# Jeffrey-Ede/AI-CV-Automation-Elect-Micr

Measured on AMD Instinct MI355X. Metric: megapixels/sec restored (512x512x1 bs=32), higher is better.
Workload: dtype bf16x3 (split-bf16 MFMA inputs, fp32 accumulate and activations)

## Files before the change

ai-cv-automation-elect-micr_amd/_lib.py:

```python
from __future__ import annotations

import ctypes as C
import os

PKG_DIR = os.path.dirname(os.path.abspath(__file__))
LIB_PATH = os.environ.get("EMD_LIB_PATH") or os.path.join(PKG_DIR, "libemdenoise.so")

EMD_OK = 0
EMD_K_SYMMETRIC = 1

_c_float_p = C.c_void_p

class PackJob(C.Structure):
    _fields_ = [("w", C.c_void_p), ("hi", C.c_void_p), ("lo", C.c_void_p), ("tap_sel", C.c_ulonglong), ("total", C.c_long),
                ("first_block", C.c_long), ("n_blocks", C.c_long), ("ntaps", C.c_int), ("cin", C.c_int), ("cout", C.c_int),
                ("cout_major", C.c_int), ("cpad", C.c_int), ("pad_", C.c_int)]


class KFusedJob(C.Structure):
    _fields_ = [("theta", C.c_void_p), ("adam_m", C.c_void_p), ("adam_v", C.c_void_p), ("step", C.c_void_p),
                ("params_out", C.c_void_p), ("losses", C.c_void_p), ("width", C.c_int), ("depth", C.c_int)]


SIGNATURES = {
# ... 336 lines not shown
    "emd_propagate_f64": (C.c_int, [C.c_void_p, C.c_int, C.c_int, C.c_int, C.c_int, C.c_void_p, C.c_double, C.c_double, C.c_double,
                                    C.c_void_p, C.c_void_p, C.c_size_t, C.c_void_p]),
    "emd_exitwave_workspace_bytes": (C.c_size_t, [C.c_int] * 3),
    "emd_exitwave_reconstruct_f64": (C.c_int, [C.c_void_p, C.c_int, C.c_int, C.c_int, C.c_void_p, C.c_double, C.c_double, C.c_double,
                                               C.c_int, C.c_int, C.c_void_p, C.c_void_p, C.c_void_p, C.c_void_p, C.c_size_t, C.c_void_p]),
    "emd_hanning_window_f64": (C.c_int, [C.c_int, C.c_void_p, C.c_void_p, C.c_void_p]),
    "emd_phase_correlate_workspace_bytes": (C.c_size_t, [C.c_int] * 3),
    "emd_phase_correlate_f64": (C.c_int, [C.c_void_p, C.c_void_p, C.c_int, C.c_int, C.c_int, C.c_void_p, C.c_void_p, C.c_void_p, C.c_size_t,
                                          C.c_void_p]),
    "emd_stack_centres_f64": (C.c_int, [C.c_void_p, C.c_int, C.c_int, C.c_void_p, C.c_void_p]),
    "emd_crop_stack_f32": (C.c_int, [C.c_void_p, C.c_int, C.c_int, C.c_void_p, C.c_int, C.c_float, C.c_void_p, C.c_void_p]),
    "emd_warp_affine_f32": (C.c_int, [C.c_void_p, C.c_int, C.c_int, C.c_int, C.c_void_p, C.c_int, C.c_float, C.c_void_p, C.c_void_p]),
    "emd_mi_samples_u32": (C.c_int, [C.c_int, C.c_int, C.c_int, C.c_uint64, C.c_void_p, C.c_void_p]),
    "emd_mattes_mi_workspace_bytes": (C.c_size_t, [C.c_int] * 5),
    "emd_mattes_mi_f64": (C.c_int, [C.c_void_p, C.c_void_p, C.c_int, C.c_int, C.c_int, C.c_void_p, C.c_void_p, C.c_int, C.c_int, C.c_void_p,
                                    C.c_void_p, C.c_void_p, C.c_void_p, C.c_size_t, C.c_void_p]),
    "emd_affine_normals_f64": (C.c_int, [C.c_int, C.c_int, C.c_int, C.c_uint64, C.c_void_p, C.c_void_p]),
    "emd_affine_register_f64": (C.c_int, [C.c_void_p, C.c_void_p, C.c_int, C.c_int, C.c_int, C.c_void_p, C.c_int, C.c_int, C.c_double,
                                          C.c_double, C.c_double, C.c_uint64, C.c_void_p, C.c_int, C.c_int, C.c_void_p, C.c_int, C.c_int,
                                          C.c_void_p, C.c_void_p, C.c_size_t, C.c_void_p]),
    "emd_affine_chain_f64": (C.c_int, [C.c_void_p, C.c_int, C.c_int, C.c_void_p, C.c_void_p]),
    "emd_affine_limits_i32": (C.c_int, [C.c_void_p, C.c_int, C.c_int, C.c_int, C.c_void_p, C.c_void_p]),
    "emd_psiart_ctf_f64": (C.c_int, [C.c_int, C.c_int, C.c_void_p, C.c_void_p, C.c_double, C.c_double, C.c_double, C.c_void_p, C.c_void_p]),
    "emd_psiart_workspace_bytes": (C.c_size_t, [C.c_int] * 2),
    "emd_psiart_loss_grad_f64": (C.c_int, [C.c_void_p, C.c_int, C.c_int] + [C.c_void_p] * 5 + [C.c_double] * 3 + [C.c_int] +
                                 [C.c_void_p] * 5 + [C.c_void_p, C.c_size_t, C.c_void_p]),
    "emd_psiart_step_f64": (C.c_int, [C.c_void_p, C.c_int, C.c_int] + [C.c_void_p] * 5 + [C.c_double] * 3 + [C.c_int] +
                            [C.c_void_p] * 8 + [C.c_double] * 3 + [C.c_void_p] * 5 + [C.c_void_p, C.c_size_t, C.c_void_p]),
}

DEV_SIGNATURES = {
    "emd_debug_knob": (C.c_int, [C.c_char_p, C.c_long]),
    "emd_debug_reduce_final_cl": (C.c_int, [C.c_int]),
    "emd_debug_split_variant": (None, [C.c_int]),
    "emd_debug_split_stamps": (None, [C.c_void_p]),
    "emd_debug_sep_stamps": (None, [C.c_void_p]),
    "emd_debug_sepgemm_stamps": (None, [C.c_void_p]),
    "emd_debug_stream_copy_f32": (C.c_int, [C.c_void_p, C.c_void_p, C.c_long, C.c_void_p]),
    "emd_debug_mfma_peak_bf16": (C.c_int, [C.c_void_p, C.c_void_p, C.c_int, C.c_int, C.c_void_p]),
}

_lib = None


class EmdError(RuntimeError):
    pass


def load():
    global _lib
    if _lib is not None:
        return _lib
    if not os.path.exists(LIB_PATH):
        raise EmdError(
            f"{LIB_PATH} not found: build the HIP extension first "
            "(python ai-cv-automation-elect-micr_amd/build.py, or __graft_entry__.build()). "
            "There is no CPU fallback for this path.")
    import torch

    lib = C.CDLL(LIB_PATH)
    for name, (res, args) in list(SIGNATURES.items()) + list(DEV_SIGNATURES.items()):
        fn = getattr(lib, name)
        fn.restype = res
        fn.argtypes = args
    _lib = lib
    for kv in filter(None, os.environ.get("EMD_KNOBS", "").split(",")):
# ... 37 lines not shown
```

ai-cv-automation-elect-micr_amd/csrc/emd_common.hip:

```cpp
#include <cstring>

#include "emd_common.hpp"

namespace emd {

static thread_local char g_err[512] = "";

void set_error(const char* fmt, ...) {
    va_list ap;
    va_start(ap, fmt);
    vsnprintf(g_err, sizeof(g_err), fmt, ap);
    va_end(ap);
}

Knobs g_knobs;

}

extern "C" int emd_version(void) { return EMD_VERSION; }

extern "C" const char* emd_last_error(void) { return emd::g_err; }

extern "C" int emd_debug_reduce_final_cl(int nslab) { return emd::reduce_final_cl(nslab); }

extern "C" int emd_debug_knob(const char* name, long value) {
    using emd::g_knobs;
    struct { const char* n; int* v; } tab[] = {
        {"sep_pipe", &g_knobs.sep_pipe}, {"sep_pipe2", &g_knobs.sep_pipe2}, {"sep_stamp_wave", &g_knobs.sep_stamp_wave}, {"sep_mode", &g_knobs.sep_mode}, {"sep_tpw", &g_knobs.sep_tpw}, {"sep_ablate", &g_knobs.sep_ablate}, {"sep_nw", &g_knobs.sep_nw}, {"sep_xcd", &g_knobs.sep_xcd},
        {"sep_wide", &g_knobs.sep_wide}, {"sep_wres", &g_knobs.sep_wres}, {"nt_mask", &g_knobs.nt_mask}, {"deconv_direct", &g_knobs.deconv_direct}, {"epi_width", &g_knobs.epi_width}, {"split_lead", &g_knobs.split_lead}, {"dw_xcd", &g_knobs.dw_xcd},
        {"dw_th", &g_knobs.dw_th},       {"split_variant", &g_knobs.split_variant}, {"split_narrow", &g_knobs.split_narrow}, {"split_wide", &g_knobs.split_wide}, {"conv3_pipe", &g_knobs.conv3_pipe}, {"wgrad_msplit", &g_knobs.wgrad_msplit}, {"wgrad_tile", &g_knobs.wgrad_tile}, {"sep_gen_pipe", &g_knobs.sep_gen_pipe}, {"fold_final", &g_knobs.fold_final}, {"up_fused", &g_knobs.up_fused}, {"exitwave_composed", &g_knobs.exitwave_composed}, {"resize_generic", &g_knobs.resize_generic},
    };
    if (!name) return -1;
    for (auto& e : tab)
        if (!strcmp(name, e.n)) { *e.v = (int)value; return 0; }
    return -1;
}
```

ai-cv-automation-elect-micr_amd/csrc/emd_common.hpp:

```cpp
#pragma once

#include <hip/hip_runtime.h>

#include <cstdarg>
#include <cstdint>
#include <cstdio>

#include "../../include/emdenoise.h"

namespace emd {

void set_error(const char* fmt, ...) __attribute__((format(printf, 1, 2)));

inline int fail(int code, const char* what) {
    set_error("%s", what);
    return code;
}

inline int check_launch(const char* kernel) {
    hipError_t e = hipGetLastError();
    if (e != hipSuccess) {
        set_error("%s: %s", kernel, hipGetErrorString(e));
        return EMD_E_LAUNCH;
    }
// ... 31 lines not shown
    bool optional;
    bool input;
};

inline int check_ranges(const char* who, const Range* r, int n, const char* aligned, const size_t* workspace_bytes = nullptr) {
    for (int i = 0; i < n; ++i)
        if (!r[i].p && !r[i].optional) {
            set_error("%s: null pointer", who);
            return EMD_E_INVALID;
        }
    if (workspace_bytes && *workspace_bytes < r[0].n) {
        set_error("%s: workspace too small (%zu bytes, needs %zu)", who, *workspace_bytes, r[0].n);
        return EMD_E_INVALID;
    }
    for (int i = 0; i < n; ++i)
        if (r[i].p && (reinterpret_cast<uintptr_t>(r[i].p) & (r[i].align - 1))) {
            set_error("%s: %s", who, aligned);
            return EMD_E_ALIGN;
        }
    for (int i = 0; i < n; ++i)
        for (int j = i + 1; j < n; ++j)
            if (r[i].p && r[j].p && !(r[i].input && r[j].input) && overlap(r[i].p, r[i].n, r[j].p, r[j].n)) {
                set_error("%s: the outputs and the workspace may overlap neither one another nor the inputs", who);
                return EMD_E_INVALID;
            }
    return EMD_OK;
}

constexpr int kWave = 64;

struct Knobs {
    int sep_pipe = 1;
    int sep_pipe2 = 0;
    int sep_gen_pipe = 0;
    int sep_mode = -1;
    int sep_nw = 0;
    int sep_ablate = 0;
    int sep_tpw = 0;
    int sep_xcd = 1;
    int sep_wide = 1;
    int sep_wres = 1;
    int fold_final = 1;
    int up_fused = 1;
    int epi_width = 0;
    int deconv_direct = 3;
    int nt_mask = 7;
    int dw_xcd = 1;
    int dw_th = 0;
    int split_narrow = 1;
    int split_lead = 2;
    int split_wide = 0;
    int conv3_pipe = 1;
    int split_variant = -1;
    int exitwave_composed = 0;
    int resize_generic = 0;
    int sep_stamp_wave = 0;
    int wgrad_msplit = 0;
    int wgrad_tile = 0;
    long long* sep_stamps = nullptr;
};
extern Knobs g_knobs;

inline long reduce_rows_per_slab(long npix) {
    long r = (npix + 511) / 512;
    return r < 64 ? 64 : r;
}
// ... 13 lines not shown
```

ai-cv-automation-elect-micr_amd/csrc/sep_fused.hip:

```cpp
#include <cstdlib>
#include <type_traits>

#include "sep_params.hpp"

using namespace emd;

namespace {

__device__ __attribute__((aligned(16))) float g_zero_px[4096];

inline int sep_nt() { return (g_knobs.nt_mask >> 1) & 1; }
inline int sep_xcd() { return g_knobs.sep_xcd; }

template <int BN, int PASSES, bool GEN, int TH = 8, bool DUAL = false, bool WRES = false>
__global__ __launch_bounds__(256, 2) void sep_fused_kernel(const SepParams p) {
    constexpr int TW = 16, BM = TH * TW, BK = 32;
    constexpr int PH = TH + 2, PW = TW + 2, NPX = PH * PW;
    constexpr int PLD = 40;
    constexpr int LDK = BK + 8;
    constexpr int WN = BN / 64, WM = 4 / WN;
    constexpr int TM = BM / WM / 32, TN = BN / WN / 32;
    constexpr int NPL = PASSES == 3 ? 2 : 1;
    constexpr int P_PASSES = (NPX * 8 + 255) / 256;
    constexpr int W_PASSES = BN / 64;
// ... 904 lines not shown

extern "C" int emd_sep3x3_fused_gen9_f32(const float* img, const float* w9, const float* gen_a, const float* gen_t, int gen_act,
                                         const float* dw, const uint16_t* whi, const uint16_t* wlo, const float* scale1,
                                         const float* shift1, const float* scale2, const float* shift2, const float* res,
                                         int ldres, float* y, int ldy, int B, int H, int W, int Cin, int Cout, int act,
                                         int precision, int reflect, emd_stream_t stream) {
    EMD_REQUIRE(img && w9 && gen_a && gen_t && dw && whi && wlo && scale1 && shift1 && y, EMD_E_INVALID,
                "emd_sep3x3_fused_gen9_f32: null pointer");
    EMD_REQUIRE((scale2 == nullptr) == (shift2 == nullptr), EMD_E_INVALID, "emd_sep3x3_fused_gen9_f32: scale2/shift2 pair");
    EMD_REQUIRE(B >= 0 && H >= 1 && W >= 1, EMD_E_INVALID, "emd_sep3x3_fused_gen9_f32: bad shape");
    EMD_REQUIRE(gen_act == EMD_ACT_RELU6 && !reflect && precision == 3 && emd_sep3x3_fused_gen9_supported(H, W, Cin, Cout),
                EMD_E_UNSUPPORTED,
                "emd_sep3x3_fused_gen9_f32: needs relu6 generation, zero padding, split-bf16, H%8==0, W%16==0, Cin 32 or 64, Cout%4==0, "
                "Cout<=64 (use emd_cin1_f32 + emd_sep3x3_fused_gen_f32)");
    EMD_REQUIRE(B <= 65535, EMD_E_UNSUPPORTED, "emd_sep3x3_fused_gen9_f32: B > 65535");
    EMD_REQUIRE(9L * W * (ldy > ldres ? ldy : ldres) < (1L << 31), EMD_E_UNSUPPORTED,
                "emd_sep3x3_fused_gen9_f32: 9 image rows of the output must span fewer than 2^31 floats");
    EMD_REQUIRE(ldy % 4 == 0 && ldy >= Cout && (!res || (ldres % 4 == 0 && ldres >= Cout)), EMD_E_ALIGN,
                "emd_sep3x3_fused_gen9_f32: pixel strides must be multiples of 4 and >= the channel count");
    EMD_REQUIRE(emd::aligned16(gen_a) && emd::aligned16(gen_t) && emd::aligned16(dw) && emd::aligned16(whi) && emd::aligned16(wlo) &&
                    emd::aligned16(y) && (!res || emd::aligned16(res)) && emd::aligned16(scale1) && emd::aligned16(shift1) &&
                    (!scale2 || (emd::aligned16(scale2) && emd::aligned16(shift2))),
                EMD_E_ALIGN, "emd_sep3x3_fused_gen9_f32: pointers (but img, w9) must be 16-byte aligned");
    if (B == 0) return EMD_OK;
    SepParams p{};
    p.x = img; p.dw = dw; p.Whi = whi; p.Wlo = wlo; p.y = y; p.res = res;
    p.scale1 = scale1; p.shift1 = shift1; p.scale2 = scale2; p.shift2 = shift2;
    p.H = H; p.W = W; p.Cin = Cin; p.Cpad = (Cin + kBK - 1) / kBK * kBK; p.N = Cout;
    p.ldx = 1; p.ldy = ldy; p.ldres = ldres; p.act = act; p.stride = 1;
    p.gen_a = gen_a; p.gen_t = gen_t; p.gen_act = gen_act; p.gen_w9 = w9;
    return launch_gen9(p, B, static_cast<hipStream_t>(stream));
}

extern "C" void emd_debug_sep_stamps(void* buf) { g_knobs.sep_stamps = static_cast<long long*>(buf); }

extern "C" int emd_sep3x3_dual_supported(int H, int W, int Cin, int Cout, int Cout2) {
    const bool wide = Cout > 64 || Cout2 > 64;
    return H % (wide ? 4 : 8) == 0 && W % 16 == 0 && Cin % 32 == 0 && Cin >= 32 && Cin <= 4096 && Cout % 4 == 0 && Cout2 % 4 == 0 &&
           Cout >= 4 && Cout2 >= 4 && Cout <= 128 && Cout2 <= 128;
}

extern "C" int emd_sep3x3_dual_preferred(int H, int W, int Cin, int Cout, int Cout2) {
    if (!emd_sep3x3_dual_supported(H, W, Cin, Cout, Cout2)) return 0;
    if (Cout <= 64 && Cout2 <= 64) return 1;
    return H % 8 == 0 && W % 32 == 0;
}

extern "C" int emd_sep3x3_dual_f32(const float* x, int ldx, const float* dw, const uint16_t* whi, const uint16_t* wlo,
                                   const float* scale1, const float* shift1, float* y, int ldy, const uint16_t* w2hi,
                                   const uint16_t* w2lo, const float* scale_b, const float* shift_b, float* y2, int ldy2, int B, int H,
                                   int W, int Cin, int Cout, int Cout2, int act, emd_stream_t stream) {
    EMD_REQUIRE(x && dw && whi && wlo && scale1 && shift1 && y && w2hi && w2lo && scale_b && shift_b && y2, EMD_E_INVALID,
                "emd_sep3x3_dual_f32: null pointer");
    EMD_REQUIRE(B >= 0 && H >= 1 && W >= 1, EMD_E_INVALID, "emd_sep3x3_dual_f32: bad shape");
    EMD_REQUIRE(emd_sep3x3_dual_supported(H, W, Cin, Cout, Cout2), EMD_E_UNSUPPORTED,
                "emd_sep3x3_dual_f32: needs H%8==0 (H%4==0 above 64 output channels), W%16==0, Cin%32==0, Cout%4==0, Cout<=128 (both outputs)");
    EMD_REQUIRE(B <= 65535, EMD_E_UNSUPPORTED, "emd_sep3x3_dual_f32: B > 65535");
    EMD_REQUIRE(9L * W * (ldy > ldy2 ? ldy : ldy2) < (1L << 31), EMD_E_UNSUPPORTED,
                "emd_sep3x3_dual_f32: 9 image rows of an output must span fewer than 2^31 floats");
    EMD_REQUIRE(ldx % 4 == 0 && ldx >= Cin && ldy % 4 == 0 && ldy >= Cout && ldy2 % 4 == 0 && ldy2 >= Cout2, EMD_E_ALIGN,
                "emd_sep3x3_dual_f32: pixel strides must be multiples of 4 and >= the channel count");
    EMD_REQUIRE(emd::aligned16(x) && emd::aligned16(dw) && emd::aligned16(whi) && emd::aligned16(wlo) && emd::aligned16(w2hi) &&
                    emd::aligned16(w2lo) && emd::aligned16(y) && emd::aligned16(y2) && emd::aligned16(scale1) && emd::aligned16(shift1) &&
                    emd::aligned16(scale_b) && emd::aligned16(shift_b),
                EMD_E_ALIGN, "emd_sep3x3_dual_f32: pointers must be 16-byte aligned");
    EMD_REQUIRE(y != y2, EMD_E_INVALID, "emd_sep3x3_dual_f32: the two outputs alias");
// ... 11 lines not shown
```

ai-cv-automation-elect-micr_amd/csrc/sep_params.hpp:

```cpp
#pragma once

#include "mfma_common.hpp"

namespace emd {

struct SepParams {
    const float* x;
    const float* dw;
    const uint16_t* Whi;
    const uint16_t* Wlo;
    float* y;
    const float* res;
    const float* scale1;
    const float* shift1;
    const float* scale2;
    const float* shift2;
    int H, W, Cin, Cpad, N;
    int ldx, ldy, ldres, act;
    int stride;
    int reflect;
    int tpw;
    const float* gen_a;
    const float* gen_t;
    int gen_act;
    int rg_stride;
    union { const uint16_t* W2hi; const float* rg_x; const float* gen_w9; };
    union { const uint16_t* W2lo; const float* fold_w; };
    union { float* y2; float* fold_z; };
    union { const float* scale_b; const float* rg_a; };
    union { const float* shift_b; const float* rg_t; };
    int N2;
    union { int ldy2; int fold; };
    int out_split;
    int rg_ld;
    long long* stamps;
    int nt;
    int ablate;
    int xcd;
    int rg_act;
};
inline bool folded(const SepParams& p) { return p.N2 == 0 && p.fold != 0; }
static_assert(sizeof(SepParams) == 232, "SepParams: the rg_* fields fill padding and share storage; see above before adding a field");

bool sep_pipe_covers(const SepParams& p, int precision);
int sep_pipe_launch(const SepParams& p, int B, hipStream_t st);
bool sep_pipe2_covers(const SepParams& p);
int sep_pipe2_launch(const SepParams& p, int B, hipStream_t st);

}
```

ai-cv-automation-elect-micr_amd/csrc/sep_pipe.hip:

```cpp
#include <type_traits>

#include "sep_params.hpp"

namespace {

using namespace emd;

__device__ __attribute__((aligned(16))) float g_zero_pipe[4096];

template <int BN, bool DUAL, int MODE, bool OSPLIT, int NW = 8, int STRIDE = 1, int EPI = 1, bool GEN = false, bool RGEN = false, bool FOLD = false>
__global__ __launch_bounds__(NW * 64, 2) void sep_pipe_kernel(const SepParams p) {
    constexpr int TW = STRIDE == 2 ? 16 : 4 * NW, TH = STRIDE == 2 ? 4 : 8, BM = TH * TW;
    constexpr int PW = STRIDE * TW + 3 - STRIDE, PH = STRIDE * TH + 3 - STRIDE, PWS = PW | 1;
    constexpr bool WPAD = PWS > PW && PH >= 9;
    constexpr int NPATCH = PH * PWS, NSLOT = WPAD ? NPATCH : NPATCH + 9;
    constexpr int WK0 = WPAD ? PW : NPATCH, WKS = WPAD ? PWS : 1;
    constexpr int NPIECE = (NSLOT + 7) / 8;
    constexpr int PP = (NPIECE + NW - 1) / NW;
    constexpr int STAGE = NPIECE * 1024;
    constexpr int A_BYTES = BM * 128, B_ONE = BN * 128;
    constexpr bool BDBL = BN <= 128 && NW == 8;
    constexpr int PB = BN / 8 / NW;
    constexpr bool LEAD2 = MODE == 0;
    constexpr int WN = STRIDE == 2 ? 4 : BN / 64, WM = NW / WN, TM = BM / WM / 32, TN = BN / WN / 32;
// ... 799 lines not shown
}

namespace emd {

static bool use_nw4(const SepParams& p) {
    if (g_knobs.sep_nw == 8 || p.stride == 2) return false;
    return p.N2 > 0 ? (p.N <= 64 && p.N2 <= 64) : (p.N <= 128 && !(p.out_split && p.N <= 64));
}

bool sep_pipe_covers(const SepParams& p, int precision) {
    if (!g_knobs.sep_pipe || precision != 3) return false;
    if (folded(p))
        return p.stride == 1 && p.H % 8 == 0 && p.W % 16 == 0 && p.Cin % 32 == 0 && p.Cin >= 32 && p.Cin <= 4064 && p.N == 64 && p.N2 == 0 &&
               !p.out_split && !p.gen_a && !p.rg_stride && !p.reflect && g_knobs.sep_nw != 8;
    if (p.gen_a)
        return g_knobs.sep_gen_pipe && p.stride == 1 && p.H % 8 == 0 && p.W % 16 == 0 && (p.Cin == 32 || p.Cin == 64) && p.N <= 64 && p.N2 == 0 &&
               !p.out_split && !p.res && g_knobs.sep_nw != 8;
    if (p.rg_stride && (p.stride != 2 || p.N2 > 0 || p.N > 128 || p.res || p.reflect)) return false;
    if (p.stride == 2)
        return p.H % 8 == 0 && p.W % 32 == 0 && p.Cin % 32 == 0 && p.Cin >= 32 && p.Cin <= 4064 && p.N2 == 0 && !p.out_split && p.N <= 256;
    if (p.H % 8 != 0 || p.W % (use_nw4(p) ? 16 : 32) != 0 || p.Cin % 32 != 0 || p.Cin < 32 || p.Cin > 4064) return false;
    if (p.N2 > 0) return p.N <= 128 && p.N2 <= 128 && !p.out_split && !p.res && !p.scale2;
    if (p.out_split && p.N <= 64) return false;
    return p.N <= 256;
}

static bool use_pipe2(const SepParams& p) {
    if (p.gen_a || p.rg_stride || folded(p)) return false;
    if (!g_knobs.sep_pipe2 || g_knobs.sep_ablate || g_knobs.sep_nw == 4 || !sep_pipe2_covers(p)) return false;
    if (g_knobs.sep_pipe2 == 2) return true;
    return p.N2 > 0 && (p.N > 64 || p.N2 > 64);
}

int sep_pipe_launch(const SepParams& p, int B, hipStream_t st) {
    if (use_pipe2(p)) return sep_pipe2_launch(p, B, st);
    SepParams q = p;
    const bool s2 = p.stride == 2;
    const int nw = (p.gen_a || folded(p) || (!s2 && use_nw4(p))) ? 4 : 8, tw = s2 ? 16 : 4 * nw, th = s2 ? 4 : 8;
    const int Ho = p.H / (s2 ? 2 : 1), Wo = p.W / (s2 ? 2 : 1);
    const int tiles_w = Wo / tw;
    const long wgs1 = (long)tiles_w * (Ho / th) * B;
    int tpw = 1;
    for (int t = 8; t >= 2; t >>= 1)
        if (tiles_w % t == 0 && wgs1 / t >= 1024 * (8 / nw)) { tpw = t; break; }
    if (g_knobs.sep_tpw > 0 && tiles_w % g_knobs.sep_tpw == 0) tpw = g_knobs.sep_tpw;
    q.tpw = tpw;
    q.stamps = g_knobs.sep_stamps;
    q.ablate = g_knobs.sep_ablate;
    const dim3 grid(tiles_w / tpw, Ho / th, B);
    q.xcd = g_knobs.sep_xcd && ((long)grid.x * grid.y * grid.z) % 8 == 0;
    const int mode = g_knobs.sep_mode >= 0 ? g_knobs.sep_mode : ((nw == 4 || p.res) ? 1 : 0);
    if (folded(p)) {
        if (mode == 1) hipLaunchKernelGGL((sep_pipe_kernel<64, false, 1, false, 4, 1, 1, false, false, true>), grid, dim3(256), 0, st, q);
        else hipLaunchKernelGGL((sep_pipe_kernel<64, false, 0, false, 4, 1, 1, false, false, true>), grid, dim3(256), 0, st, q);
        return emd::check_launch("sep_pipe_kernel<folded final conv>");
    }
    if (p.gen_a) {
        if (g_knobs.epi_width == 4) hipLaunchKernelGGL((sep_pipe_kernel<64, false, 1, false, 4, 1, 4, true>), grid, dim3(256), 0, st, q);
        else hipLaunchKernelGGL((sep_pipe_kernel<64, false, 1, false, 4, 1, 1, true>), grid, dim3(256), 0, st, q);
        return emd::check_launch("sep_pipe_kernel<generated input>");
    }
    if (p.rg_stride) {
        hipLaunchKernelGGL((sep_pipe_kernel<128, false, 1, false, 8, 2, 1, false, true>), grid, dim3(512), 0, st, q);
        return emd::check_launch("sep_pipe_kernel<stride 2, generated residual>");
    }
    const int epi = g_knobs.epi_width ? g_knobs.epi_width : ((p.res && p.N > 128) ? 4 : 1);
    return epi == 4 ? launch_epi<4>(p, q, grid, mode, nw, st) : launch_epi<1>(p, q, grid, mode, nw, st);
}
// ... 3 lines not shown
```

ai-cv-automation-elect-micr_amd/csrc/sep_pipe2.hip:

```cpp
#include "sep_params.hpp"

namespace {

using namespace emd;

__device__ __attribute__((aligned(16))) float g_zero_pipe2[4096];

typedef __attribute__((ext_vector_type(2))) float f32x2v;

template <int BN, bool DUAL, bool OSPLIT, int EPI>
__global__ __launch_bounds__(512, 2) void sep_pipe2_kernel(const SepParams p) {
    constexpr int NW = 8, TW = 32, TH = 8, BM = TH * TW;
    constexpr int PW = TW + 2, PH = TH + 2, PWS = PW | 1;
    constexpr int NPATCH = PH * PWS, NSLOT = NPATCH;
    constexpr int WK0 = PW, WKS = PWS;
    constexpr int NPIECE = (NSLOT + 7) / 8, PP = (NPIECE + NW - 1) / NW, STAGE = NPIECE * 1024;
    constexpr int A_HALF = BM * 64, B_HALF = BN * 64;
    constexpr int A_OFF = 2 * STAGE, B_OFF = A_OFF + 2 * A_HALF, C_OFF = B_OFF + 2 * B_HALF, SMEM = C_OFF + 16 * BN;
    constexpr int NBP = BN / 16;
    constexpr int PB = NBP >= NW ? NBP / NW : 1;
    constexpr int WN = BN / 64, WM = NW / WN, TM = BM / WM / 32, TN = 2;
    constexpr int E = 16 / EPI * TM * TN;
    constexpr bool RPRE = TM == 1 && !DUAL;
    constexpr int R = RPRE ? 16 / EPI * TM * TN : 0;
    static_assert(SMEM <= 160 * 1024 && PP >= 2, "shape");
    static_assert(!(DUAL && OSPLIT), "split32 output: one-output instances only");
    __shared__ __attribute__((aligned(1024))) unsigned char smem[SMEM];

    const int tid = threadIdx.x, lane = tid & 63;
    const int wv = __builtin_amdgcn_readfirstlane(tid >> 6);
    int wm, wn;
    if constexpr (DUAL) {
// ... 494 lines not shown
        PIPE_STAMP(0)
        slot_body(odd, stg, !epi_here, dq);
        if (s == -1 && !out2) zero_acc();
        PIPE_STAMP(1)
        wait_lgkm0();
        PIPE_STAMP(2)
        if (odd) {
            if (k < 0 || (!full && (epi_last || rp))) wait_vm<0>();
            else if (epi_last) wait_vm<PP + E>();
            else if (rp) wait_vm<PP + R>();
            else wait_vm<PP>();
        } else {
            if (epi_last && full) wait_vm<E>();
            else wait_vm<0>();
        }
        PIPE_STAMP(3)
        __builtin_amdgcn_s_barrier();
        PIPE_STAMP(4)
        if (!odd) {
            if (last0) x_epi += TW;
            ct1 = ct2;
            ++k;
        }
    }
    wait_vm<0>();
    if (p.stamps && tid == p.ablate * 64) {
        long long* o = p.stamps + ((long)(blockIdx.z * gridDim.y + blockIdx.y) * gridDim.x + blockIdx.x) * 8;
#pragma unroll
        for (int i = 0; i < 8; ++i) o[i] = ph[i];
    }
#undef PIPE_STAMP
}

template <int BN, bool DUAL, bool OSPLIT, int EPI>
int launch2(const SepParams& q, dim3 grid, hipStream_t st) {
    hipLaunchKernelGGL((sep_pipe2_kernel<BN, DUAL, OSPLIT, EPI>), grid, dim3(512), 0, st, q);
    return emd::check_launch("sep_pipe2_kernel");
}

}

namespace emd {

bool sep_pipe2_covers(const SepParams& p) {
    if (p.stride != 1 || p.gen_a || p.H % 8 != 0 || p.W % 32 != 0 || p.Cin % 32 != 0 || p.Cin < 32 || p.Cin > 4064) return false;
    if (p.N2 > 0) return p.N <= 128 && p.N2 <= 128 && !p.out_split && !p.res && !p.scale2;
    if (p.out_split && p.N <= 64) return false;
    return p.N <= 256;
}

int sep_pipe2_launch(const SepParams& p, int B, hipStream_t st) {
    SepParams q = p;
    const int tiles_w = p.W / 32;
    const long wgs1 = (long)tiles_w * (p.H / 8) * B;
    int tpw = 1;
    for (int t = 8; t >= 2; t >>= 1)
        if (tiles_w % t == 0 && wgs1 / t >= 1024) { tpw = t; break; }
    if (g_knobs.sep_tpw > 0 && tiles_w % g_knobs.sep_tpw == 0) tpw = g_knobs.sep_tpw;
    q.tpw = tpw;
    q.stamps = g_knobs.sep_stamps;
    q.ablate = g_knobs.sep_stamp_wave & 7;
    const dim3 grid(tiles_w / tpw, p.H / 8, B);
    q.xcd = g_knobs.sep_xcd && ((long)grid.x * grid.y * grid.z) % 8 == 0;
    const int epi = g_knobs.epi_width ? g_knobs.epi_width : ((p.res && p.N > 128) ? 4 : 1);
    if (p.N2 > 0) {
        if (p.N > 64 || p.N2 > 64) return launch2<256, true, false, 1>(q, grid, st);
        return launch2<128, true, false, 1>(q, grid, st);
    }
    if (p.N <= 64) return launch2<64, false, false, 1>(q, grid, st);
    if (p.N <= 128) return p.out_split ? launch2<128, false, true, 1>(q, grid, st) : launch2<128, false, false, 1>(q, grid, st);
    if (p.out_split) return epi == 4 ? launch2<256, false, true, 4>(q, grid, st) : launch2<256, false, true, 1>(q, grid, st);
    return epi == 4 ? launch2<256, false, false, 4>(q, grid, st) : launch2<256, false, false, 1>(q, grid, st);
}

}
```

include/emdenoise_dev.h:

```cpp
#ifndef EMDENOISE_DEV_H
#define EMDENOISE_DEV_H
#ifdef __cplusplus
extern "C" {
#endif

int emd_debug_knob(const char* name, long value);
int emd_debug_reduce_final_cl(int nslab);
void emd_debug_split_variant(int v);
void emd_debug_split_stamps(void* device_buf);
void emd_debug_sep_stamps(void* device_buf);
void emd_debug_sepgemm_stamps(void* device_buf);


int emd_debug_stream_copy_f32(const float* src, float* dst, long n, void* stream);
int emd_debug_mfma_peak_bf16(const void* ops, float* out, int workgroups, int iters, void* stream);

#ifdef __cplusplus
}
#endif
#endif
```

Baseline: 392.5.

## Add chunked pipelined dual-output separable conv kernel with warp-specialized roles

Adds a new sep_pipe2_chunk kernel for dual-output separable 3x3 convolutions where one output exceeds 64 channels. Four waves compute the depthwise stage and main GEMM, while the other four run the second-output GEMM from the patch center. The patch, B-weight and epilogue loads are pipelined across Cin chunks and tiles. It is enabled by default through kChunkRule and routed before the old path, trading extra kernel complexity and LDS state for better overlap on these shapes.

Result: faster. 399.4 (median of 6 runs) (+1.8%).

```diff
diff --git a/ai-cv-automation-elect-micr_amd/_lib.py b/ai-cv-automation-elect-micr_amd/_lib.py
--- a/ai-cv-automation-elect-micr_amd/_lib.py
+++ b/ai-cv-automation-elect-micr_amd/_lib.py
@@ -392,6 +392,7 @@
 DEV_SIGNATURES = {
     "emd_debug_knob": (C.c_int, [C.c_char_p, C.c_long]),
     "emd_debug_reduce_final_cl": (C.c_int, [C.c_int]),
+    "emd_debug_sep_pipe2_chunk_covers": (C.c_int, [C.c_int] * 5),
     "emd_debug_split_variant": (None, [C.c_int]),
     "emd_debug_split_stamps": (None, [C.c_void_p]),
     "emd_debug_sep_stamps": (None, [C.c_void_p]),
diff --git a/ai-cv-automation-elect-micr_amd/csrc/emd_common.hip b/ai-cv-automation-elect-micr_amd/csrc/emd_common.hip
--- a/ai-cv-automation-elect-micr_amd/csrc/emd_common.hip
+++ b/ai-cv-automation-elect-micr_amd/csrc/emd_common.hip
@@ -26,7 +26,7 @@
 extern "C" int emd_debug_knob(const char* name, long value) {
     using emd::g_knobs;
     struct { const char* n; int* v; } tab[] = {
-        {"sep_pipe", &g_knobs.sep_pipe}, {"sep_pipe2", &g_knobs.sep_pipe2}, {"sep_stamp_wave", &g_knobs.sep_stamp_wave}, {"sep_mode", &g_knobs.sep_mode}, {"sep_tpw", &g_knobs.sep_tpw}, {"sep_ablate", &g_knobs.sep_ablate}, {"sep_nw", &g_knobs.sep_nw}, {"sep_xcd", &g_knobs.sep_xcd},
+        {"sep_pipe", &g_knobs.sep_pipe}, {"sep_pipe2", &g_knobs.sep_pipe2}, {"sep_pipe2_chunk", &g_knobs.sep_pipe2_chunk}, {"sep_stamp_wave", &g_knobs.sep_stamp_wave}, {"sep_mode", &g_knobs.sep_mode}, {"sep_tpw", &g_knobs.sep_tpw}, {"sep_ablate", &g_knobs.sep_ablate}, {"sep_nw", &g_knobs.sep_nw}, {"sep_xcd", &g_knobs.sep_xcd},
         {"sep_wide", &g_knobs.sep_wide}, {"sep_wres", &g_knobs.sep_wres}, {"nt_mask", &g_knobs.nt_mask}, {"deconv_direct", &g_knobs.deconv_direct}, {"epi_width", &g_knobs.epi_width}, {"split_lead", &g_knobs.split_lead}, {"dw_xcd", &g_knobs.dw_xcd},
         {"dw_th", &g_knobs.dw_th},       {"split_variant", &g_knobs.split_variant}, {"split_narrow", &g_knobs.split_narrow}, {"split_wide", &g_knobs.split_wide}, {"conv3_pipe", &g_knobs.conv3_pipe}, {"wgrad_msplit", &g_knobs.wgrad_msplit}, {"wgrad_tile", &g_knobs.wgrad_tile}, {"sep_gen_pipe", &g_knobs.sep_gen_pipe}, {"fold_final", &g_knobs.fold_final}, {"up_fused", &g_knobs.up_fused}, {"exitwave_composed", &g_knobs.exitwave_composed}, {"resize_generic", &g_knobs.resize_generic},
     };
diff --git a/ai-cv-automation-elect-micr_amd/csrc/emd_common.hpp b/ai-cv-automation-elect-micr_amd/csrc/emd_common.hpp
--- a/ai-cv-automation-elect-micr_amd/csrc/emd_common.hpp
+++ b/ai-cv-automation-elect-micr_amd/csrc/emd_common.hpp
@@ -87,6 +87,7 @@
 struct Knobs {
     int sep_pipe = 1;
     int sep_pipe2 = 0;
+    int sep_pipe2_chunk = -1;
     int sep_gen_pipe = 0;
     int sep_mode = -1;
     int sep_nw = 0;
diff --git a/ai-cv-automation-elect-micr_amd/csrc/sep_fused.hip b/ai-cv-automation-elect-micr_amd/csrc/sep_fused.hip
--- a/ai-cv-automation-elect-micr_amd/csrc/sep_fused.hip
+++ b/ai-cv-automation-elect-micr_amd/csrc/sep_fused.hip
@@ -960,6 +960,13 @@
     return launch_gen9(p, B, static_cast<hipStream_t>(stream));
 }
 
+extern "C" int emd_debug_sep_pipe2_chunk_covers(int H, int W, int Cin, int Cout, int Cout2) {
+    if (!emd_sep3x3_dual_supported(H, W, Cin, Cout, Cout2)) return 0;
+    emd::SepParams p{};
+    p.H = H; p.W = W; p.Cin = Cin; p.N = Cout; p.N2 = Cout2; p.stride = 1;
+    return emd::sep_pipe2_chunk_covers(p) ? 1 : 0;
+}
+
 extern "C" void emd_debug_sep_stamps(void* buf) { g_knobs.sep_stamps = static_cast<long long*>(buf); }
 
 extern "C" int emd_sep3x3_dual_supported(int H, int W, int Cin, int Cout, int Cout2) {
diff --git a/ai-cv-automation-elect-micr_amd/csrc/sep_params.hpp b/ai-cv-automation-elect-micr_amd/csrc/sep_params.hpp
--- a/ai-cv-automation-elect-micr_amd/csrc/sep_params.hpp
+++ b/ai-cv-automation-elect-micr_amd/csrc/sep_params.hpp
@@ -46,5 +46,7 @@
 int sep_pipe_launch(const SepParams& p, int B, hipStream_t st);
 bool sep_pipe2_covers(const SepParams& p);
 int sep_pipe2_launch(const SepParams& p, int B, hipStream_t st);
+bool sep_pipe2_chunk_covers(const SepParams& p);
+int sep_pipe2_chunk_launch(const SepParams& p, int B, hipStream_t st);
 
 }
diff --git a/ai-cv-automation-elect-micr_amd/csrc/sep_pipe.hip b/ai-cv-automation-elect-micr_amd/csrc/sep_pipe.hip
--- a/ai-cv-automation-elect-micr_amd/csrc/sep_pipe.hip
+++ b/ai-cv-automation-elect-micr_amd/csrc/sep_pipe.hip
@@ -855,8 +855,16 @@
     return p.N2 > 0 && (p.N > 64 || p.N2 > 64);
 }
 
+constexpr int kChunkRule = 1;
+static bool use_pipe2_chunk(const SepParams& p) {
+    const int on = g_knobs.sep_pipe2_chunk < 0 ? kChunkRule : g_knobs.sep_pipe2_chunk;
+    if (!on || g_knobs.sep_pipe2 || g_knobs.sep_ablate || g_knobs.sep_nw == 4 || g_knobs.sep_stamps) return false;
+    return sep_pipe2_chunk_covers(p);
+}
+
 int sep_pipe_launch(const SepParams& p, int B, hipStream_t st) {
     if (use_pipe2(p)) return sep_pipe2_launch(p, B, st);
+    if (use_pipe2_chunk(p)) return sep_pipe2_chunk_launch(p, B, st);
     SepParams q = p;
     const bool s2 = p.stride == 2;
     const int nw = (p.gen_a || folded(p) || (!s2 && use_nw4(p))) ? 4 : 8, tw = s2 ? 16 : 4 * nw, th = s2 ? 4 : 8;
diff --git a/ai-cv-automation-elect-micr_amd/csrc/sep_pipe2.hip b/ai-cv-automation-elect-micr_amd/csrc/sep_pipe2.hip
--- a/ai-cv-automation-elect-micr_amd/csrc/sep_pipe2.hip
+++ b/ai-cv-automation-elect-micr_amd/csrc/sep_pipe2.hip
@@ -1,3 +1,5 @@
+#include <type_traits>
+
 #include "sep_params.hpp"
 
 namespace {
@@ -558,6 +560,423 @@
 #undef PIPE_STAMP
 }
 
+template <int EPI>
+__global__ __launch_bounds__(512, 2) void sep_pipe2_chunk_kernel(const SepParams p) {
+    constexpr int BN = 256, NW = 8, TW = 32, TH = 8, BM = TH * TW;
+    constexpr int PW = TW + 2, PH = TH + 2, PWS = PW | 1;
+    constexpr int NPATCH = PH * PWS, NSLOT = NPATCH;
+    constexpr int WK0 = PW, WKS = PWS;
+    constexpr int NPIECE = (NSLOT + 7) / 8, PP = (NPIECE + NW - 1) / NW, STAGE = NPIECE * 1024;
+    constexpr int A_HALF = BM * 64, B_HALF = BN * 64;
+    constexpr int A_OFF = 2 * STAGE, B_OFF = A_OFF + 2 * A_HALF, C_OFF = B_OFF + 2 * B_HALF, P_OFF = C_OFF + 8 * BN, SMEM = P_OFF + 128;
+    constexpr int NBP = BN / 16, PB = NBP / NW;
+    constexpr int WN = BN / 64, WM = NW / WN, TM = BM / WM / 32, TN = 2;
+    constexpr int E = 16 / EPI * TM * TN;
+    static_assert(SMEM <= 160 * 1024 && PP >= 2 && PB >= 1 && TM == 4, "shape");
+    __shared__ __attribute__((aligned(1024))) unsigned char smem[SMEM];
+
+    const int tid = threadIdx.x, lane = tid & 63;
+    const int wv = __builtin_amdgcn_readfirstlane(tid >> 6);
+    const int idx = wv & 3, wm = idx % WM, wn = (wv >> 2) * (WN / 2) + idx / WM;
+    int bx = blockIdx.x, by = blockIdx.y, bz = blockIdx.z;
+    xcd_remap(p.xcd, bx, by, bz);
+    const int xbase = bx * p.tpw * TW;
+    enum { L_X = 0, L_DW = 8, L_Y = 16, L_Y2 = 24, L_LDY = 32, L_LDY2 = 36, L_N = 40, L_N2 = 44, L_ACT = 48, L_H = 52, L_W = 56, L_CIN = 60, L_LDX = 64,
+           L_REFLECT = 68, L_Y0 = 72, L_BZ = 76 };
+    if (tid == 0) {
+        unsigned char* l = smem + P_OFF;
+        *reinterpret_cast<const float**>(l + L_X) = p.x;
+        *reinterpret_cast<const float**>(l + L_DW) = p.dw;
+        *reinterpret_cast<float**>(l + L_Y) = p.y;
+        *reinterpret_cast<float**>(l + L_Y2) = p.y2;
+        *reinterpret_cast<int*>(l + L_LDY) = p.ldy;
+        *reinterpret_cast<int*>(l + L_LDY2) = p.ldy2;
+        *reinterpret_cast<int*>(l + L_N) = p.N;
+        *reinterpret_cast<int*>(l + L_N2) = p.N2;
+        *reinterpret_cast<int*>(l + L_ACT) = p.act;
+        *reinterpret_cast<int*>(l + L_H) = p.H;
+        *reinterpret_cast<int*>(l + L_W) = p.W;
+        *reinterpret_cast<int*>(l + L_CIN) = p.Cin;
+        *reinterpret_cast<int*>(l + L_LDX) = p.ldx;
+        *reinterpret_cast<int*>(l + L_REFLECT) = p.reflect;
+        *reinterpret_cast<int*>(l + L_Y0) = by * TH;
+        *reinterpret_cast<int*>(l + L_BZ) = bz;
+    }
+    __syncthreads();
+    auto lds_i = [&](int off) { return __builtin_amdgcn_readfirstlane(*reinterpret_cast<const int*>(smem + P_OFF + off)); };
+    auto lds_p = [&](int off) {
+        const unsigned lo = lds_i(off), hi = lds_i(off + 4);
+        return reinterpret_cast<float*>(((unsigned long long)hi << 32) | lo);
+    };
+
+    const float* psrc[PP];
+    unsigned pmove = 0;
+    auto set_tile = [&](int xt) {
+        int drow = lane >> 3, dk = lane & 7, w = wv;
+        asm volatile("" : "+v"(drow), "+v"(dk), "+s"(w));
+        pmove = 0;
+        const float* px_ = lds_p(L_X);
+        const float* pdw = lds_p(L_DW);
+        const int H = lds_i(L_H), W = lds_i(L_W), Cin = lds_i(L_CIN), ldx = lds_i(L_LDX), reflect = lds_i(L_REFLECT), y0 = lds_i(L_Y0);
+        const long img = (long)lds_i(L_BZ) * H * W;
+#pragma unroll
+        for (int j = 0; j < PP; ++j) {
+            int q = w + NW * j;
+            if (q >= NPIECE) q -= NW;
+            const int slot = q * 8 + drow;
+            const int py = slot / PWS, px = slot - py * PWS;
+            int gy = y0 - 1 + py, gx = xt - 1 + px;
+            if (reflect) {
+                gy = gy < 0 ? -gy : (gy >= H ? 2 * H - 2 - gy : gy);
+                gx = gx < 0 ? -gx : (gx >= W ? 2 * W - 2 - gx : gx);
+            }
+            const bool real = slot < NPATCH && px < PW && gy >= 0 && gy < H && gx >= 0 && gx < W;
+            const bool wk = slot < NPATCH && px == PW && py < 9;
+            const int kk = dk ^ ((px >> 1) & 7);
+            const float* o = g_zero_pipe2 + dk * 4;
+            const float* o_px = px_ + (img + (long)gy * W + gx) * ldx + kk * 4;
+            const float* o_wk = pdw + (long)py * Cin + dk * 4;
+            o = real ? o_px : o;
+            o = wk ? o_wk : o;
+            psrc[j] = o;
+            pmove |= real ? 1u << j : 0u;
+        }
+    };
+    auto issue_patch = [&](int stage, int coff, int j0 = 0, int j1 = PP) {
+#pragma unroll
+        for (int j = j0; j < j1; ++j) {
+            int q = wv + NW * j;
+            if (q >= NPIECE) q -= NW;
+            __builtin_amdgcn_global_load_lds((gptr_t)(psrc[j] + coff), (lptr_t)(smem + stage * STAGE + q * 1024), 16, 0, 0);
+        }
+    };
+    const uint16_t* bsrc[PB];
+    int bq[PB];
+    bool bproj[PB];
+#pragma unroll
+    for (int j = 0; j < PB; ++j) {
+        const int q = (wv * PB + j) % NBP;
+        const int row = q * 16 + (lane >> 2);
+        const int c = (lane & 3) ^ ((row >> 2) & 3);
+        const bool second = row >= BN / 2;
+        const int rr = second ? row - BN / 2 : row;
+        const uint16_t* plane = (c & 2) ? (second ? p.W2lo : p.Wlo) : (second ? p.W2hi : p.Whi);
+        bsrc[j] = plane + (long)rr * p.Cpad + (c & 1) * 8;
+        bq[j] = q;
+        bproj[j] = q >= NBP / 2;
+    }
+    auto issue_B = [&](int hm, int cm, int hp, int cp) {
+#pragma unroll
+        for (int j = 0; j < PB; ++j) {
+            const int h = bproj[j] ? hp : hm, c = bproj[j] ? cp : cm;
+            __builtin_amdgcn_global_load_lds((gptr_t)(bsrc[j] + c + h * 16), (lptr_t)(smem + B_OFF + h * B_HALF + bq[j] * 1024), 16, 0, 0);
+        }
+    };
+
+    const bool full = p.N == BN / 2 && p.N2 == BN / 2;
+    const int nchunks = p.Cin / 32;
+    const int total = p.tpw * nchunks;
+    int istep = 0, ic = 0, ixt = xbase;
+    set_tile(xbase);
+    auto advance_issue = [&]() {
+        if (istep + 1 >= total) return;
+        ++istep;
+        if (++ic == nchunks) {
+            ic = 0;
+            const int xn = ixt + TW;
+            if (ixt >= 1 && xn + TW + 1 <= p.W) {
+                const long step = (long)TW * p.ldx;
+#pragma unroll
+                for (int j = 0; j < PP; ++j) psrc[j] += ((pmove >> j) & 1) ? step : 0;
+            } else {
+                set_tile(xn);
+            }
+            ixt = xn;
+        }
+    };
+
+    if (tid < BN) {
+        const bool second = tid >= BN / 2;
+        const int nn = second ? tid - BN / 2 : tid;
+        const bool valid = nn < (second ? p.N2 : p.N);
+        float* cst = reinterpret_cast<float*>(smem + C_OFF);
+        cst[tid] = valid ? (second ? p.scale_b : p.scale1)[nn] : 0.f;
+        cst[BN + tid] = valid ? (second ? p.shift_b : p.shift1)[nn] : 0.f;
+    }
+
+    issue_B(1, 0, 0, 0);
+    issue_patch(0, 0);
+    advance_issue();
+    issue_patch(1, ic * 32);
+    wait_vm<PP>();
+    __builtin_amdgcn_s_barrier();
+
+    auto role = [&](auto out2c) {
+        constexpr bool OUT2 = decltype(out2c)::value;
+        const int fr = lane & 31, fh = lane >> 5, gf = (fr >> 2) & 3;
+        const int row0 = wm * TM * 32;
+        const int qd = lane & 3, cell = (lane >> 2) & 7;
+        const int st = (((cell >> 2) ^ (cell >> 1) ^ cell) & 1) + 2 * (lane >> 5);
+        const int dy = 2 * idx + (cell & 1), dx = 4 * (st & 1) + 16 * (st >> 1) + 8 * ((cell >> 1) & 1);
+        int rdv[3];
+#pragma unroll
+        for (int m = 0; m < 3; ++m) rdv[m] = (dy * PWS + dx) * 128 + ((qd ^ (((dx >> 1) + m) & 7)) << 4);
+        const int wk_off = WK0 * 128 + qd * 16;
+        const int a_wr = A_OFF + (dy * TW + dx) * 64 + (((qd >> 1) ^ ((dx >> 2) & 3)) << 4) + (qd & 1) * 8;
+        const int a_wr2 = a_wr ^ 32;
+        const int a_rd = A_OFF + (row0 + fr) * 64 + ((fh ^ gf) << 4), a_rd2 = a_rd ^ 32;
+        const int cen = ((row0 / TW + 1) * PWS + fr + 1) * 128 + (((fh * 2) ^ (((fr + 1) >> 1) & 7)) << 4);
+        const int b_rd = B_OFF + (wn * 64 + fr) * 64 + ((fh ^ gf) << 4), b_rd2 = b_rd ^ 32;
+
+        f32x16 acc[TM][TN];
+        auto zero_acc = [&]() {
+#pragma unroll
+            for (int i = 0; i < TM; ++i)
+#pragma unroll
+                for (int j = 0; j < TN; ++j)
+#pragma unroll
+                    for (int e = 0; e < 16; ++e) acc[i][j][e] = 0.f;
+        };
+        zero_acc();
+
+        auto epilogue = [&](int x0) {
+            int fr = lane & 31, fh = lane >> 5;
+            asm volatile("" : "+v"(fr), "+v"(fh));
+            int actc = OUT2 ? 1 : lds_i(L_ACT);
+            const float hi = actc == 1 ? 6.f : __builtin_inff();
+            const float slope = actc == 4 ? 0.2f : 1.f, lo = (actc == 1 || actc == 2) ? 0.f : -__builtin_inff();
+            const bool simple = actc == 1;
+            float* __restrict__ outp = lds_p(OUT2 ? L_Y2 : L_Y);
+            const int ldo = lds_i(OUT2 ? L_LDY2 : L_LDY), nlim = lds_i(OUT2 ? L_N2 : L_N), wo = lds_i(L_W);
+            int yrow = row0 / TW;
+            asm volatile("" : "+s"(yrow));
+            yrow += lds_i(L_Y0);
+            const long imgo = (long)lds_i(L_BZ) * lds_i(L_H) * wo;
+            float es1[TN], et1[TN];
+#pragma unroll
+            for (int j = 0; j < TN; ++j) {
+                const float* cst = reinterpret_cast<const float*>(smem + C_OFF) + wn * 64 + j * 32 + fr;
+                es1[j] = cst[0];
+                et1[j] = cst[BN];
+            }
+            const int li = fr & 3, cq = fr >> 2;
+            unsigned voff[TN];
+            bool live[TN];
+#pragma unroll
+            for (int j = 0; j < TN; ++j) {
+                const int nb = wn * 64 + j * 32 - (OUT2 ? BN / 2 : 0);
+                const int n = EPI == 1 ? nb + fr : nb + 4 * cq;
+                live[j] = n < nlim;
+                voff[j] = EPI == 1 ? (unsigned)(4 * fh * ldo + n) * 4u : (unsigned)((4 * fh + li) * ldo + n) * 4u;
+            }
+#pragma unroll
+            for (int i = 0; i < TM; ++i) {
+                const long pixr = imgo + (long)(yrow + i) * wo + x0;
+                float* obase = outp + pixr * ldo;
+#pragma unroll
+                for (int q = 0; q < 4; ++q) {
+                    float r[TN][4];
+#pragma unroll
+                    for (int j = 0; j < TN; ++j) {
+                        const float s1 = es1[j], t1 = et1[j];
+                        if constexpr (EPI == 1) {
+                            if (simple) {
+#pragma unroll
+                                for (int k = 0; k < 4; ++k) r[j][k] = __builtin_amdgcn_fmed3f(fmaf(acc[i][j][4 * q + k], s1, t1), 0.f, 6.f);
+                            } else {
+#pragma unroll
+                                for (int k = 0; k < 4; ++k) {
+                                    const float u = fmaf(acc[i][j][4 * q + k], s1, t1);
+                                    r[j][k] = __builtin_amdgcn_fmed3f(fmaxf(u, slope * u), lo, hi);
+                                }
+                            }
+                        } else {
+                            if (simple) {
+#pragma unroll
+                                for (int k = 0; k < 4; ++k) r[j][k] = fminf(fmaxf(fmaf(acc[i][j][4 * q + k], s1, t1), 0.f), 6.f);
+                            } else {
+#pragma unroll
+                                for (int k = 0; k < 4; ++k) {
+                                    const float u = fmaf(acc[i][j][4 * q + k], s1, t1);
+                                    r[j][k] = fminf(fmaxf(fmaxf(u, lo), slope * u), hi);
+                                }
+                            }
+                            quad_transpose(r[j], li);
+                        }
+                    }
+                    if constexpr (EPI == 1) {
+#pragma unroll
+                        for (int k = 0; k < 4; ++k) {
+                            float* ob = obase + (8 * q + k) * ldo;
+#pragma unroll
+                            for (int j = 0; j < TN; ++j)
+                                if (live[j]) store_nt_d(ob, voff[j], __builtin_bit_cast(unsigned, r[j][k]));
+                        }
+                    } else {
+                        float* ob = obase + 8 * q * ldo;
+#pragma unroll
+                        for (int j = 0; j < TN; ++j)
+                            if (live[j]) store_nt_s(ob, voff[j], f32x4{r[j][0], r[j][1], r[j][2], r[j][3]});
+                    }
+                }
+            }
+            zero_acc();
+        };
+
+        auto body = [&](auto oddc, const int stg, const bool patch, const int pstage, const int pcoff) {
+            constexpr int ODD = decltype(oddc)::value;
+            constexpr int HS = 1 - ODD, HM = OUT2 ? 1 - ODD : ODD;
+            const int fa_1 = OUT2 ? stg + (cen ^ (HM * 64)) : a_rd, fa_2 = OUT2 ? stg + (cen ^ (HM * 64) ^ 16) : a_rd2;
+            constexpr int FA_IMM = OUT2 ? 0 : HM * A_HALF, FSTRIDE = OUT2 ? PWS * 128 : 2048;
+            const int swk = stg + wk_off;
+            int srd[3];
+#pragma unroll
+            for (int m = 0; m < 3; ++m) srd[m] = stg + (rdv[m] ^ (HS * 64));
+            f32x4 wk[3], pr[6], o[4];
+            auto rd_row = [&](int i) {
+                if constexpr (!OUT2) {
+#pragma unroll
+                    for (int d = 0; d < 3; ++d) wk[d] = *reinterpret_cast<const f32x4*>(smem + swk + HS * 64 + (i * 3 + d) * (WKS * 128));
+#pragma unroll
+                    for (int d = 0; d < 6; ++d) pr[d] = *reinterpret_cast<const f32x4*>(smem + srd[d >> 1] + (i * PWS + d) * 128);
+                }
+            };
+            auto fma_row = [&]() {
+                if constexpr (!OUT2) {
+#pragma unroll
+                    for (int j = 0; j < 4; ++j)
+#pragma unroll
+                        for (int d = 0; d < 3; ++d) o[j] += wk[d] * pr[j + d];
+                    asm volatile("" : "+v"(o[0]), "+v"(o[1]), "+v"(o[2]), "+v"(o[3]));
+                }
+            };
+            bf16x8 bh[TN], bl[TN];
+            u32x4 f0[TM], f1[TM];
+            auto ld_b = [&]() {
+#pragma unroll
+                for (int j = 0; j < TN; ++j) {
+                    bh[j] = *reinterpret_cast<const bf16x8*>(smem + b_rd + HM * B_HALF + j * 2048);
+                    bl[j] = *reinterpret_cast<const bf16x8*>(smem + b_rd2 + HM * B_HALF + j * 2048);
+                }
+            };
+            auto ld_a = [&](int i) {
+                f0[i] = *reinterpret_cast<const u32x4*>(smem + fa_1 + FA_IMM + i * FSTRIDE);
+                f1[i] = *reinterpret_cast<const u32x4*>(smem + fa_2 + FA_IMM + i * FSTRIDE);
+            };
+            auto cvt_a = [&](int i) {
+                if constexpr (OUT2) {
+                    const f32x4 v0 = __builtin_bit_cast(f32x4, f0[i]), v1 = __builtin_bit_cast(f32x4, f1[i]);
+                    unsigned h0, h1, h2, h3, l0, l1, l2, l3;
+                    split2(v0[0], v0[1], h0, l0);
+                    split2(v0[2], v0[3], h1, l1);
+                    split2(v1[0], v1[1], h2, l2);
+                    split2(v1[2], v1[3], h3, l3);
+                    f0[i] = u32x4{h0, h1, h2, h3};
+                    f1[i] = u32x4{l0, l1, l2, l3};
+                }
+            };
+            auto mm = [&](int i, int j) {
+                const bf16x8 ah = __builtin_bit_cast(bf16x8, f0[i]), al = __builtin_bit_cast(bf16x8, f1[i]);
+                acc[i][j] = __builtin_amdgcn_mfma_f32_32x32x16_bf16(al, bh[j], acc[i][j], 0, 0, 0);
+                acc[i][j] = __builtin_amdgcn_mfma_f32_32x32x16_bf16(ah, bl[j], acc[i][j], 0, 0, 0);
+                acc[i][j] = __builtin_amdgcn_mfma_f32_32x32x16_bf16(ah, bh[j], acc[i][j], 0, 0, 0);
+            };
+            auto seg_mm = [&](int i) {
+                cvt_a(i);
+#pragma unroll
+                for (int j = 0; j < TN; ++j) mm(i, j);
+            };
+            if constexpr (!OUT2) {
+#pragma unroll
+                for (int j = 0; j < 4; ++j) o[j] = f32x4{0.f, 0.f, 0.f, 0.f};
+            }
+            constexpr int P3 = (PP + 2) / 3;
+            ld_b();
+            ld_a(0);
+            rd_row(0);
+            __builtin_amdgcn_sched_barrier(0);
+            seg_mm(0);
+            fma_row();
+            rd_row(1);
+            ld_a(1);
+            if (patch) issue_patch(pstage, pcoff, 0, P3);
+            __builtin_amdgcn_sched_barrier(0);
+            seg_mm(1);
+            fma_row();
+            rd_row(2);
+            ld_a(2);
+            if (patch) issue_patch(pstage, pcoff, P3, 2 * P3 < PP ? 2 * P3 : PP);
+            __builtin_amdgcn_sched_barrier(0);
+            seg_mm(2);
+            fma_row();
+            ld_a(3);
+            if (patch) issue_patch(pstage, pcoff, 2 * P3 < PP ? 2 * P3 : PP, PP);
+            __builtin_amdgcn_sched_barrier(0);
+            seg_mm(3);
+            if constexpr (!OUT2) {
+#pragma unroll
+                for (int j = 0; j < 4; ++j) {
+                    unsigned h0, l0, h1, l1;
+                    split2(o[j][0], o[j][1], h0, l0);
+                    split2(o[j][2], o[j][3], h1, l1);
+                    *reinterpret_cast<u32x2*>(smem + a_wr + HS * A_HALF + j * 64) = u32x2{h0, h1};
+                    *reinterpret_cast<u32x2*>(smem + a_wr2 + HS * A_HALF + j * 64) = u32x2{l0, l1};
+                }
+            }
+            __builtin_amdgcn_sched_barrier(0);
+        };
+
+        int k = -1, ct1 = 0, x_epi = xbase;
+        auto slot = [&](auto oddc, auto epic) {
+            constexpr int ODD = decltype(oddc)::value;
+            constexpr bool MAYEPI = decltype(epic)::value && (ODD != 0) == OUT2;
+            const int stg = ((k + 1) & 1) * STAGE;
+            const int ct2 = ct1 + 1 == nchunks ? 0 : ct1 + 1;
+            const bool last0 = k >= 0 && ct1 == 0;
+            const bool epi_here = MAYEPI && last0;
+            const bool patch = ODD && k >= 0;
+            const int pstage = k & 1;
+            if (patch) advance_issue();
+            const int pcoff = ic * 32;
+            issue_B(ODD ? 0 : 1, ct1 * 32, ODD ? 1 : 0, (ODD ? ct1 : ct2) * 32);
+            if constexpr (MAYEPI) {
+                if (epi_here) {
+                    if (patch) issue_patch(pstage, pcoff);
+                    epilogue(x_epi);
+                }
+            }
+            body(oddc, stg, patch && !epi_here, pstage, pcoff);
+            wait_lgkm0();
+            if constexpr (ODD) {
+                if (k < 0 || (!full && epi_here)) wait_vm<0>();
+                else if (epi_here) wait_vm<PP + E>();
+                else wait_vm<PP>();
+            } else {
+                if (epi_here && full) wait_vm<E>();
+                else wait_vm<0>();
+            }
+            __builtin_amdgcn_s_barrier();
+            if constexpr (!ODD) {
+                if (last0) x_epi += TW;
+                ct1 = ct2;
+                ++k;
+            }
+        };
+        using C0 = std::integral_constant<int, 0>;
+        using C1 = std::integral_constant<int, 1>;
+        slot(C1{}, std::false_type{});
+        if constexpr (!OUT2) zero_acc();
+        for (int t = 0; t < total; ++t) {
+            slot(C0{}, std::true_type{});
+            slot(C1{}, std::true_type{});
+        }
+        slot(C0{}, std::true_type{});
+    };
+    if (wv < 4) role(std::false_type{});
+    else role(std::true_type{});
+    wait_vm<0>();
+}
+
 template <int BN, bool DUAL, bool OSPLIT, int EPI>
 int launch2(const SepParams& q, dim3 grid, hipStream_t st) {
     hipLaunchKernelGGL((sep_pipe2_kernel<BN, DUAL, OSPLIT, EPI>), grid, dim3(512), 0, st, q);
@@ -599,4 +1018,27 @@
     return epi == 4 ? launch2<256, false, false, 4>(q, grid, st) : launch2<256, false, false, 1>(q, grid, st);
 }
 
+bool sep_pipe2_chunk_covers(const SepParams& p) {
+    if (p.stride != 1 || p.gen_a || p.rg_stride || p.H % 8 != 0 || p.W % 32 != 0 || p.Cin % 32 != 0 || p.Cin < 32 || p.Cin > 4064) return false;
+    return p.N2 > 0 && p.N <= 128 && p.N2 <= 128 && (p.N > 64 || p.N2 > 64) && !p.out_split && !p.res && !p.scale2;
 }
+
+int sep_pipe2_chunk_launch(const SepParams& p, int B, hipStream_t st) {
+    SepParams q = p;
+    const int tiles_w = p.W / 32;
+    const long wgs1 = (long)tiles_w * (p.H / 8) * B;
+    int tpw = 1;
+    for (int t = 8; t >= 2; t >>= 1)
+        if (tiles_w % t == 0 && wgs1 / t >= 1024) { tpw = t; break; }
+    if (g_knobs.sep_tpw > 0 && tiles_w % g_knobs.sep_tpw == 0) tpw = g_knobs.sep_tpw;
+    q.tpw = tpw;
+    q.stamps = nullptr;
+    q.ablate = 0;
+    const dim3 grid(tiles_w / tpw, p.H / 8, B);
+    q.xcd = g_knobs.sep_xcd && ((long)grid.x * grid.y * grid.z) % 8 == 0;
+    if (g_knobs.epi_width == 4) hipLaunchKernelGGL((sep_pipe2_chunk_kernel<4>), grid, dim3(512), 0, st, q);
+    else hipLaunchKernelGGL((sep_pipe2_chunk_kernel<1>), grid, dim3(512), 0, st, q);
+    return emd::check_launch("sep_pipe2_chunk_kernel");
+}
+
+}
diff --git a/include/emdenoise_dev.h b/include/emdenoise_dev.h
--- a/include/emdenoise_dev.h
+++ b/include/emdenoise_dev.h
@@ -6,6 +6,7 @@
 
 int emd_debug_knob(const char* name, long value);
 int emd_debug_reduce_final_cl(int nslab);
+int emd_debug_sep_pipe2_chunk_covers(int H, int W, int Cin, int Cout, int Cout2);
 void emd_debug_split_variant(int v);
 void emd_debug_split_stamps(void* device_buf);
 void emd_debug_sep_stamps(void* device_buf);
```
